# viq854/bwbble

Hardware: AMD Instinct MI355X
Metric: 100bp reads aligned/sec (inexact BWT backward search, IUPAC FM-index) (higher is better)
Workload: dtype u64

## Files before the change

### bwbble_amd/csrc/bwb_hip.hip

```cpp
#include <hip/hip_runtime.h>
#include <time.h>
#include <algorithm>
#include <cctype>
#include <cmath>
#include <cstdio>
#include <cstdlib>
#include <cstring>
#include <memory>
#include <string>
#include <thread>
#include <vector>
#include "../../include/bwbble_hip.h"
#include "bwb_kernels.h"
static double wall_s() { struct timespec ts; clock_gettime(CLOCK_MONOTONIC, &ts); return ts.tv_sec + 1e-9 * ts.tv_nsec; }
#include "bwb_lane.h"

static thread_local std::string g_err;
static int fail(int code, const std::string &m) { g_err = m; return code; }
#define HIPCHK(x)                                                                                         \
	do {                                                                                                  \
		hipError_t e_ = (x);                                                                              \
		if (e_ != hipSuccess) return fail(BWB_E_HIP, std::string(#x) + ": " + hipGetErrorString(e_));  \
	} while (0)

// ... 23 lines not shown
	hipError_t reserve(size_t n) {
		if (p && bytes >= n) return hipSuccess;
		if (p) (void)hipHostFree(p);
		p = nullptr; bytes = 0;
		hipError_t e = hipHostMalloc(&p, n ? n : 1, hipHostMallocDefault);
		if (e == hipSuccess) bytes = n; else p = nullptr;
		return e;
	}
	template <typename T> T *as() const { return (T *)p; }
};
struct Event {
	hipEvent_t e = nullptr;
	Event() = default;
	Event(const Event &) = delete;
	Event &operator=(const Event &) = delete;
	~Event() { if (e) (void)hipEventDestroy(e); }
	hipError_t create() { return e ? hipSuccess : hipEventCreate(&e); }
};

struct AltBufs {
	DevMem d_cnt, d_off, d_bsum, d_alts;
	PinMem h_off, h_alts;
};

struct ScratchClass {
	DevMem mem;
	LaneScratch sc{};
	uint32_t blocks = 0;
	bool ready = false;
};

struct Slot {
	bool uploaded = false, submitted = false, complete = false, fetched = false;
	uint32_t n_reads = 0, stride = 0, maxlen = 0, dstride = 0;
	DevMem d_reads, d_lens, d_dbuf, d_status, d_n, d_off, d_worklist, d_log, d_ctl, d_dbg_iters, d_src;
	uint32_t n_tot = 0;
	bool inherit = false;
	std::vector<uint32_t> h_src;
	uint64_t log_cap = 0;
	PinMem h_reads, h_lens, h_cnt, h_off, h_log, h_ctl;
	DevMem d_place;
	PinMem h_place;
	int placed_mm = -1;
	AltBufs alt;
	int placed_alt = -1;
	std::vector<uint8_t> h_status;
	std::vector<uint64_t> h_aln_off;
	std::vector<bwb_aln> h_alns;
	Event ev_up;
	bool calcd_queued = false;
	Event ev_calcd;
	uint64_t launch = 0;
	uint32_t *ctl_counter() const { return d_ctl.as<uint32_t>(); }
	unsigned int *ctl_done() const { return d_ctl.as<unsigned int>() + 16; }
	unsigned long long *ctl_count() const { return (unsigned long long *)(d_ctl.as<unsigned char>() + 128); }
	uint32_t *ctl_counter2() const { return d_ctl.as<uint32_t>() + 48; }
};

struct PendingTime { hipEvent_t e0, e1; int kind; };

struct bwb_hip_ctx {
	int device = 0, num_cu = 0;
	hipStream_t stream = nullptr, cstream = nullptr, rstream = nullptr;
	hipStream_t dstream = nullptr;
	int calcd_ahead = 0;
	DevIndex ix{};
	DevMem d_buckets, d_SA, d_stats, d_descs, d_misc;
// ... 436 lines not shown
	c->p = *p; c->have_params = true;
	c->kp = KParams{ p->max_diff, p->max_gapo, p->max_gape, p->max_entries, p->mm_score, p->gapo_score, p->gape_score,
	                 p->seed_length, p->max_diff_seed, p->max_best, p->no_indel_length, nb, p->use_precalc ? 1 : 0, p->is_multiref ? 1 : 0 };
	c->wide = wide;

	uint32_t maxlen = 0, n_bad = 0;
	const uint32_t sl = (uint32_t)p->seed_length;
	auto is_source = [&](const uint8_t *seq, uint32_t len) {
		if (!(sl && len > sl) || len > 255) return false;
		if (p->use_precalc) { if (len < PRECALC_LEN) return false; for (int k = 0; k < PRECALC_LEN; k++) if (seq[k] > 3) return false; }
		return true;
	};
	const bool ghost = carry_seq && is_source(carry_seq, carry_len) && n_reads;
	uint32_t last = ghost ? n_reads : NONE32;
	s.inherit = false;
	s.h_src.clear();
	for (uint32_t i = 0; i < n_reads; i++) {
		const bool bad = lens[i] > 255 || lens[i] > stride || (p->use_precalc && lens[i] < PRECALC_LEN);
		if (bad) { n_bad++; continue; }
		maxlen = std::max<uint32_t>(maxlen, lens[i]);
		if (is_source(reads_fwd + (size_t)i * stride, lens[i])) last = i;
		else if (sl && lens[i] <= sl && last != NONE32) {
			if (!s.inherit) { s.h_src.assign(n_reads, NONE32); s.inherit = true; }
			s.h_src[i] = last;
		}
	}
	const bool use_ghost = ghost && s.inherit;
	if (s.inherit && !use_ghost) for (uint32_t i = 0; i < n_reads; i++) if (s.h_src[i] == n_reads) s.h_src[i] = NONE32;
	if (s.inherit) { bool any = false; for (uint32_t v : s.h_src) any |= v != NONE32; s.inherit = any; }
	if (use_ghost) maxlen = std::max<uint32_t>(maxlen, carry_len);
	s.n_tot = n_reads + (use_ghost && s.inherit ? 1u : 0u);
	if (n_bad) fprintf(stderr, "[bwbble_hip] warning: %u read(s) longer than 255 bases%s get an empty alignment record\n", n_bad, p->use_precalc ? " or shorter than 12 (-P)" : "");
	s.n_reads = n_reads; s.stride = std::min<uint32_t>(stride, std::max<uint32_t>(maxlen, 1)); s.maxlen = maxlen;
	s.dstride = REC_BYTES * rec_count(maxlen) + 16;
	const size_t nr = s.n_tot ? s.n_tot : 1;
	HIPCHK(s.d_reads.reserve(nr * s.stride));
	HIPCHK(s.d_lens.reserve(nr * 2));
	HIPCHK(s.d_dbuf.reserve(nr * s.dstride));
	HIPCHK(s.d_status.reserve(nr));
	HIPCHK(s.d_worklist.reserve(nr * 4));
	HIPCHK(s.d_n.reserve(nr * 4));
	HIPCHK(s.d_off.reserve(nr * 8));
	HIPCHK(s.d_ctl.reserve(256));
	HIPCHK(s.h_ctl.reserve(256));
	HIPCHK(s.ev_up.create());
	const uint64_t want = std::max<uint64_t>((uint64_t)nr * 8, 1u << 16);
	if (s.log_cap < want) { HIPCHK(s.d_log.alloc(want * sizeof(bwb_aln))); s.log_cap = want; }
	if (c->dbg_iters) { HIPCHK(s.d_dbg_iters.reserve(nr * 4)); HIPCHK(hipMemsetAsync(s.d_dbg_iters.p, 0, nr * 4, c->cstream)); }
	HIPCHK(s.h_reads.reserve(nr * s.stride));
	HIPCHK(s.h_lens.reserve(nr * 2));
	uint8_t *hr = s.h_reads.as<uint8_t>();
	uint16_t *hl = s.h_lens.as<uint16_t>();
	if (s.stride == stride && !n_bad) { memcpy(hr, reads_fwd, (size_t)n_reads * stride); memcpy(hl, lens, (size_t)n_reads * 2); }
	else
		for (uint32_t i = 0; i < n_reads; i++) {
			const bool bad = lens[i] > 255 || lens[i] > stride || (p->use_precalc && lens[i] < PRECALC_LEN);
			hl[i] = bad ? (uint16_t)BAD_LEN : lens[i];
			memcpy(hr + (size_t)i * s.stride, reads_fwd + (size_t)i * stride, bad ? 0 : lens[i]);
		}
	if (s.n_tot > n_reads) { hl[n_reads] = (uint16_t)carry_len; memcpy(hr + (size_t)n_reads * s.stride, carry_seq, carry_len); }
	if (s.n_tot) {
		HIPCHK(hipMemcpyAsync(s.d_reads.p, hr, (size_t)s.n_tot * s.stride, hipMemcpyHostToDevice, c->cstream));
		HIPCHK(hipMemcpyAsync(s.d_lens.p, hl, (size_t)s.n_tot * 2, hipMemcpyHostToDevice, c->cstream));
	}
	if (s.inherit) {
		HIPCHK(s.d_src.reserve((size_t)n_reads * 4));
		HIPCHK(hipMemcpyAsync(s.d_src.p, s.h_src.data(), (size_t)n_reads * 4, hipMemcpyHostToDevice, c->cstream));
		HIPCHK(hipStreamSynchronize(c->cstream));
	}
	SlotDesc &d = c->h_descs[si];
	d.b.reads = s.d_reads.as<uint8_t>(); d.b.lens = s.d_lens.as<uint16_t>(); d.b.n_reads = n_reads; d.b.stride = s.stride;
	d.b.dbuf = s.d_dbuf.as<uint8_t>(); d.b.dstride = s.dstride; d.b.status = s.d_status.as<uint8_t>(); d.b.dbg_iters = s.d_dbg_iters.as<uint32_t>();
	d.out.alns = s.d_log.as<uint4>(); d.out.count = s.ctl_count(); d.out.cap = s.log_cap; d.out.off = s.d_off.as<uint64_t>(); d.out.n = s.d_n.as<uint32_t>();
	d.done = s.ctl_done();
	HIPCHK(hipMemcpyAsync(c->d_descs.as<SlotDesc>() + si, &d, sizeof(SlotDesc), hipMemcpyHostToDevice, c->cstream));
	HIPCHK(hipEventRecord(s.ev_up.e, c->cstream));
	s.uploaded = true; s.submitted = false; s.complete = false; s.fetched = false; s.placed_mm = -1; s.placed_alt = -1;
	return ensure_class(c, 0);
}

template <typename P> static DTab<P> dtab_of(const bwb_hip_ctx *c) {
	DTab<P> t;
	const bool use = c->dtab_K > 0 && c->dtab_multiref == (c->kp.multiref ? 1 : 0);
	t.ent = use ? c->d_dtab_ent.as<uint4>() : nullptr;
	t.pool = c->d_dtab_pool.as<Intv<P>>();
	t.K = c->dtab_K;
	for (int j = 0; j < 4; j++) t.nm1[j] = c->dtab_nm1[j];
	return t;
}

#define DTAB_MIN_READS 200000u
static bool any_in_flight(const bwb_hip_ctx *c);
template <typename P> static int build_dtab_t(bwb_hip_ctx *c, int K) {
	const double t0 = wall_s();
	ScratchClass &sc = c->cls[0];
	const size_t isz = sizeof(Intv<P>);
	const size_t need_half = std::min<size_t>((size_t)64 << 24, (size_t)(c->ix.length + c->ix.length / 2) + ((size_t)1 << (2 * K))) * isz;
	DevMem tmp;
	unsigned char *pool0 = c->d_pool.as<unsigned char>();
	size_t half = (c->d_pool.bytes / 2) & ~(size_t)255;
	if (half < need_half) {
		if (tmp.alloc(2 * need_half) == hipSuccess) { pool0 = tmp.as<unsigned char>(); half = need_half; }
		else (void)hipGetLastError();
	}
	const unsigned long long cap = half / isz;
// ... 168 lines not shown
		float ms = 0;
		HIPCHK(hipEventElapsedTime(&ms, e0, e1));
		unsigned int hb[POOL_REGIONS * 16], used_max = 0;
		unsigned long long used = 0;
		int rc = fetch(c, hb, bump, sizeof(hb));
		if (rc) return rc;
		const uint32_t priv = (grid + s.sc.n_regions - 1) / s.sc.n_regions * LANE_BLOCK * s.sc.keep;
		for (uint32_t r = 0; r < s.sc.n_regions; r++) { used += std::min(priv + hb[r * 16], s.sc.pool_cap); used_max = std::max(used_max, priv + hb[r * 16]); }
		fprintf(stderr, "[bwb] kl_search class %d slot %d: %u new reads, grid %u, %s%s, %.3f ms, pool chunks used %llu of %d x %u (fullest region asked for %u; %u private per lane)\n",
		        k, si, n_work, grid, suspend ? "slice (parks)" : "drains", resume ? ", resumes parked reads" : "", ms, used, (int)s.sc.n_regions, s.sc.pool_cap, used_max, s.sc.keep);
	}
	if (c->launch_log) return log_launch(c, "kl_search", k, si, !(suspend || slice_iters != 0), c->stream, e0, e1);
	return BWB_OK;
}

static int queue_calc_d(bwb_hip_ctx *c, int si) {
	Slot &s = c->slots[si];
	HIPCHK(s.ev_calcd.create());
	HIPCHK(hipStreamWaitEvent(c->dstream, s.ev_up.e, 0));
	HIPCHK(hipMemsetAsync(s.d_status.p, 0, (size_t)s.n_tot, c->dstream));
	int rc = launch_calc_d(c, 0, si, nullptr, s.n_tot, s.ctl_counter(), nullptr, nullptr, c->dstream);
	if (rc) return rc;
	rc = launch_inherit(c, si, c->dstream);
	if (rc) return rc;
	HIPCHK(hipEventRecord(s.ev_calcd.e, c->dstream));
	s.calcd_queued = true;
	return BWB_OK;
}

static int submit(bwb_hip_ctx *c, int si, bool suspend) {
	Slot &s = c->slots[si];
	if (!s.uploaded) return fail(BWB_E_STATE, "slot_submit: nothing uploaded into this slot");
	if (s.submitted && !s.complete) return fail(BWB_E_STATE, "slot_submit: the slot is still in flight");
	int rc = index_ready(c);
	if (rc) return rc;
	rc = ensure_class(c, 0);
	if (rc) return rc;
	rc = ensure_dtab(c, s.n_reads);
	if (rc) return rc;
	HIPCHK(hipStreamWaitEvent(c->stream, s.ev_up.e, 0));
	const bool ahead = c->calcd_ahead > 0 && s.n_reads != 0;
	if (ahead) {
		if (!s.calcd_queued) { rc = queue_calc_d(c, si); if (rc) return rc; }
		HIPCHK(hipStreamWaitEvent(c->stream, s.ev_calcd.e, 0));
	}
	HIPCHK(hipMemsetAsync(s.d_ctl.p, 0, 256, c->stream));
	s.submitted = true; s.complete = false; s.fetched = false; s.placed_mm = -1; s.placed_alt = -1; s.launch = 0;
	if (s.n_reads == 0) { s.complete = true; s.launch = c->n_launches; return BWB_OK; }
	HIPCHK(hipMemsetAsync(s.d_n.p, 0, (size_t)s.n_reads * 4, c->stream));
	if (!ahead) {
		HIPCHK(hipMemsetAsync(s.d_status.p, 0, (size_t)s.n_tot, c->stream));
		rc = launch_calc_d(c, 0, si, nullptr, s.n_tot, s.ctl_counter(), nullptr, nullptr);
		if (rc) return rc;
		rc = launch_inherit(c, si);
		if (rc) return rc;
	}
	rc = launch_search(c, 0, si, nullptr, s.n_reads, s.ctl_counter(), suspend);
	if (rc) return rc;
	s.launch = c->n_launches;
	for (int k = 1; ahead && k <= c->calcd_ahead; k++) {
		const int sj = (si + k) % BWB_MAX_SLOTS;
		Slot &t = c->slots[sj];
		if (t.uploaded && !t.submitted && !t.calcd_queued && t.n_reads) { rc = queue_calc_d(c, sj); if (rc) return rc; }
	}
	return BWB_OK;
}
// ... 697 lines not shown
```

### bwbble_amd/csrc/bwb_kernels.h

```cpp
#pragma once
#include "bwb_device.h"

#define BWB_BLOCK 256
#define BWB_OCTS_PER_BLOCK 32
#define NONE32 0xFFFFFFFFu
#define BAD_LEN 0xFFFFu
#define ST_OK 0
#define ST_SCRATCH_OVF 1
#define ST_OUT_OVF 2
#define ST_D_OVF 3
#define ST_D_WAIT 4

struct KParams {
	int max_diff, max_gapo, max_gape, max_entries;
	int mm_score, gapo_score, gape_score;
	int seed_length, max_diff_seed, max_best, no_indel_length;
	int num_buckets;
	int use_precalc;
	int multiref;
};

struct Batch {
	const uint8_t *reads;
	const uint16_t *lens;
	uint32_t n_reads, stride;
	uint8_t *dbuf;
	uint32_t dstride;
	uint8_t *status;
	uint32_t *dbg_iters;
};

struct OutBuf {
	uint4 *alns;
	unsigned long long *count;
	uint64_t cap;
	uint64_t *off;
	uint32_t *n;
};

struct SlotDesc {
	Batch b;
	OutBuf out;
	unsigned int *done;
};

struct Work {
	const uint32_t *worklist;
	uint32_t n_work;
	uint32_t *counter;
	uint32_t slot;
	uint32_t suspend;
	uint32_t slice_iters;
	uint32_t resume;
};

enum { STAT_VIS_SINGLE = 0, STAT_VIS_ALPHA, STAT_POPS, STAT_PUSHES, STAT_ALNS, STAT_N, STAT_N_MAX, STAT_VIS_CALCD,
       STAT_BKT_SEARCH , STAT_BKT_CALCD, STAT_PARKED ,
       STAT_ENT_ST , STAT_ENT_LD , STAT_REC_LD ,
       STAT_WAVE_ITERS = 16, STAT_WAVE_ITERS_CALCD = 17, STAT_LOCATE_STEPS = 18 , STAT_STAMPS = 24, STAT_HIST = 40 , STAT_BBPROF = 104 ,
#ifdef BWB_BBPROF
       STAT_WORDS = 104 + 2048 };
#else
       STAT_WORDS = 104 };
#endif

template <typename P> struct Intv { P L, U; };

#define REC_BYTES 16
__host__ __device__ __forceinline__ uint32_t rec_count(uint32_t len) { return (len >> 2) + 1u; }
__device__ __forceinline__ void rec_put(uint8_t *recs, uint32_t nrec, int arr, int k, uint32_t v) {
	const int m = (k + 2) >> 2, t = (k + 2) & 3;
	if ((uint32_t)m < nrec) recs[REC_BYTES * m + arr + t] = (uint8_t)v;
	if (t < 2 && m > 0) recs[REC_BYTES * (m - 1) + arr + 4 + t] = (uint8_t)v;
}
__device__ __forceinline__ uint32_t rec_get(const uint8_t *recs, int arr, int k) { return recs[REC_BYTES * ((k + 2) >> 2) + arr + ((k + 2) & 3)]; }

__device__ __forceinline__ uint32_t single_mask_codes(int c) { return c == 0 ? 1u << 15 : (c == 1 ? 1u << 3 : (c == 2 ? 1u << 7 : 1u << 1)); }
__device__ __forceinline__ uint32_t member_mask(int c) {
	return c == 0 ? 0xFB00u : (c == 1 ? 0x383Cu : (c == 2 ? 0x0BF0u : 0x6266u));
}

template <typename P> __device__ __forceinline__ void load_base(P *s_base, const DevIndex &ix) {
	for (int t = threadIdx.x; t < BWB_BASE_ROWS * 16; t += BWB_BLOCK) s_base[t] = (P)ix.base[t >> 4][t & 15];
	__syncthreads();
}
template <typename P> __device__ __forceinline__ void load_base2(P *s_base, const DevIndex &ix) {
	for (int t = threadIdx.x; t < BWB_BASE_ROWS * 16; t += BWB_BLOCK) {
		const int row = t >> 4, j = t & 15;
		const P v = (P)ix.base[row][j];
		s_base[t] = v;
		if (row < BWB_NSB_MAX) s_base[BWB_BASE_ROWS * 16 + t] = ((0x2A20u >> j) & 1u) ? (P)(ix.base[BWB_ROW_NEG][j] - 1) : v;
	}
	__syncthreads();
}

__global__ void k_relayout(const uint32_t *bwt, const uint64_t *O, uint64_t blk0, uint64_t nblk_chunk, uint64_t nwords_chunk, uint64_t sa0_index,
                           const uint64_t *sbcount , uint4 *buckets) {
	const uint64_t t = (uint64_t)blockIdx.x * blockDim.x + threadIdx.x;
	if (t >= nblk_chunk * 8) return;
	const uint64_t lb = t >> 3, blk = blk0 + lb;
	const int sl = (int)(t & 7);
	const uint64_t w0 = lb * 16;
	uint4 o;
	if (sl < 4) {
		const uint32_t first = w0 < nwords_chunk ? (bwt[w0] >> 28) : 0u;
		const uint64_t *row = O + lb * 16;
		const uint64_t *sb = sbcount + (blk >> BWB_SB_SHIFT) * 16;
		const int cs[4] = { 2 * sl, 2 * sl + 1, 2 * sl + 8, 2 * sl + 9 };
// ... 84 lines not shown
			uint64_t x = (q + u) * 0x9E3779B97F4A7C15ull + seed;
			x ^= x >> 29; x *= 0xBF58476D1CE4E5B9ull; x ^= x >> 32;
			rank_issue<P>(ix.buckets, (P)(ix.length - 1), (P)(x % (ix.length - 1)), ol, rq[u]);
		}
#pragma unroll
		for (int u = 0; u < 4; u++) {
			P v0, v1;
			rank_finish<P, false>(rq[u], s_base, ol, lane, v0, v1);
			acc += (ol == 0 ? 0ull : (unsigned long long)v0) + 3ull * v1;
		}
	}
	acc += __shfl_xor(acc, 1); acc += __shfl_xor(acc, 2); acc += __shfl_xor(acc, 4);
	if (ol == 0 && acc) atomicAdd(checksum, acc);
}

__global__ void k_gather(const uint4 *log, const uint64_t *off, const uint32_t *n, const uint64_t *dst_off, uint32_t n_reads, uint4 *dst) {
	const uint32_t rid = blockIdx.x * (blockDim.x >> 3) + (threadIdx.x >> 3);
	if (rid >= n_reads) return;
	const int ol = threadIdx.x & 7;
	const uint64_t so = off[rid] * 2, d = dst_off[rid] * 2;
	const uint32_t cnt = n[rid] * 2;
	for (uint32_t t = ol; t < cnt; t += 8) dst[d + t] = log[so + t];
}

__global__ void k_dseed_inherit(Batch b, const uint32_t *src, uint32_t n) {
	const uint32_t r = blockIdx.x * blockDim.x + threadIdx.x;
	if (r >= n) return;
	const uint32_t q = src[r];
	if (q == NONE32) return;
	if (b.status[q] == ST_D_OVF) { if (b.status[r] != ST_D_OVF) b.status[r] = ST_D_WAIT; return; }
	const int lr = b.lens[r], lq = b.lens[q];
	uint8_t *rr = b.dbuf + (size_t)r * b.dstride;
	const uint8_t *rq = b.dbuf + (size_t)q * b.dstride;
	for (int k = -2; k < lr; k++) rec_put(rr, rec_count((uint32_t)lr), 8, k, rec_get(rq, 8, k + lq - lr));
	if (b.status[r] == ST_D_WAIT) b.status[r] = ST_OK;
}

__device__ __forceinline__ uint64_t sa_walk(const DevIndex &ix, const uint64_t *s_base, uint64_t sa0_index, uint64_t i, int lane, int ol, uint64_t &j) {
	while ((i & 31) != 0) {
		if (i == sa0_index) { i = 0; j++; continue; }
		RankReq<uint64_t> ra;
		rank_issue<uint64_t>(ix.buckets, ix.length - 1, i, ol, ra);
		const uint4 cq = ra.regular ? ra.q : ix.buckets[(i >> BKT_SHIFT) * 8 + ol];
		const int off = (int)(i & BKT_MASK), srcl = (lane & ~7) + 4 + (off >> 5), bit = off & 31;
		const uint32_t code_here = ((cq.x >> bit) & 1u) | (((cq.y >> bit) & 1u) << 1) | (((cq.z >> bit) & 1u) << 2) | (((cq.w >> bit) & 1u) << 3);
		const uint32_t code = oct_bcast(code_here, srcl);
		uint64_t v0, v1;
		rank_finish<uint64_t, false>(ra, s_base, ol, lane, v0, v1);
		const uint64_t mine = (code & 1u) ? v1 : v0;
		uint64_t nxt = oct_bcast(mine, (lane & ~7) + (int)(code >> 1));
		if (code == 0 && ra.regular && sa0_index >= (i & ~127ull) && sa0_index <= i) nxt--;
		i = nxt;
		j++;
	}
	return i;
}

__global__ __launch_bounds__(BWB_BLOCK) void k_locate(DevIndex ix, const uint64_t *SA, uint64_t sa0_index, const uint64_t *rows, uint64_t n, uint64_t *out, unsigned long long *stats) {
	__shared__ uint64_t s_base[BWB_BASE_ROWS * 16];
	load_base<uint64_t>(s_base, ix);
	const int lane = threadIdx.x & 63, ol = lane & 7;
	const uint64_t noct = (uint64_t)gridDim.x * BWB_OCTS_PER_BLOCK;
	for (uint64_t q = (uint64_t)blockIdx.x * BWB_OCTS_PER_BLOCK + (threadIdx.x >> 3); q < n; q += noct) {
		uint64_t j = 0;
		const uint64_t i = sa_walk(ix, s_base, sa0_index, rows[q], lane, ol, j);
		if (ol == 0) { out[q] = (SA[i >> 5] + j) % ix.length; if (j) atomicAdd(&stats[STAT_LOCATE_STEPS], (unsigned long long)j); }
	}
// ... 223 lines not shown
```

### bwbble_amd/csrc/bwb_lane.h

```cpp
#pragma once
#include "bwb_device.h"
#include "bwb_kernels.h"

#define LANE_BLOCK 256
#ifndef LANE_WAVES_PER_SIMD
#define LANE_WAVES_PER_SIMD 3
#endif
template <typename P> using Lds = __attribute__((address_space(3))) P *;
__device__ __forceinline__ unsigned long long wballot(bool b) { return __builtin_amdgcn_ballot_w64(b); }
__device__ __forceinline__ bool wany(bool b) { return __builtin_amdgcn_ballot_w64(b) != 0ull; }
__device__ __forceinline__ bool wall(bool b) { return __builtin_amdgcn_ballot_w64(!b) == 0ull; }
#define CHUNK_SLOTS 64
#define POOL_REGIONS 8
#define BSTATE_ROW_MIN 128
#define PRECALC_LEN 12
#define ADMIT_CHUNKS 1024
#define SAVE_U4 16
#define ALN_U4 3

struct LaneScratch {
	uint4 *pool;
	size_t region_u4;
	uint32_t n_regions;
	unsigned int *pool_bump;
// ... 419 lines not shown
                                                        uint32_t dbg_ld, uint32_t dbg_lds, unsigned long long *stats, DTab<P> dt) {
	extern __shared__ __align__(16) unsigned char smem_[];
	const LdsBytes smem = (LdsBytes)(uintptr_t)(((uint32_t)(uintptr_t)(LdsBytes)smem_ + 127u) & ~127u);
	P *s_base = (P *)smem;
	const int lane = (int)(threadIdx.x & 63u);
	LdsBytes wlds = smem + CALCD_WAVES_OFF + (threadIdx.x >> 6) * WAVE_LDS_BYTES_NU(CALCD_NU);
	Lds<u32x4> stage = (Lds<u32x4>)wlds, zero_row = (Lds<u32x4>)(smem + CALCD_ZERO_OFF);
	const Lds<P> sb = (Lds<P>)smem;
	if (threadIdx.x < 32) ((Lds<uint32_t>)zero_row)[threadIdx.x] = 0u;
	load_base<P>(s_base, ix);
	const uint32_t slot = blockIdx.x * LANE_BLOCK + threadIdx.x;
	Intv<P> *lbase = (Intv<P> *)sc.lists_d + (size_t)slot * 2 * sc.lcap;
	const int cap = (int)sc.lcap;
	const uint4 *__restrict__ buckets = ix.buckets;
	const P last_row = (P)(ix.length - 1);

	bool active = false, done = false;
	uint32_t rid = 0;
	int len = 0, phase = 0, plen = 0, r = 0, z = 0, s = 0, curT = 0, cursel = 0;
	Intv<P> nxi; nxi.L = nxi.U = 0; bool nxi_valid = false;
	typedef IntvRegs<P> IR;
	typename IR::W g0 = {}, g1 = {}, g2 = {}, g3 = {};
	int cg = -1;
	int c = 4, cnext = 4;
	P cL = 0, cU = 0;
	ListW<P> nx; nx.T = 0; nx.tL = nx.tU = 0; nx.fL = nx.fU = 0;
	ListBuf<P> wb; wb.b0 = wb.b1 = wb.b2 = wb.b3 = typename IntvRegs<P>::W{};
	int32_t nm = 0, prev_nm = 0;
	uint32_t bacc = 0, cntN = 0;
	unsigned long long vis = 0;
	uint32_t r_vis = 0, n_bkt = 0;
	const uint8_t *seq = b.reads;
	const Intv<P> *curb = lbase;
	auto from_table = [&]() -> bool {
		if (!dt.ent || dbgD || r < dt.K) return false;
		unsigned long long idx = 0;
		bool ok = true;
		for (int t = 0; t < dt.K; t++) { const uint32_t ch = seq[r - t]; ok &= ch <= 3u; idx |= (unsigned long long)(ch & 3u) << (2 * t); }
		if (!ok) return false;
		const uint4 ea = dt.ent[2 * idx], eb = dt.ent[2 * idx + 1];
		const int T = (int)dtab_T(ea);
		if (!dtab_valid(ea) || T + 15 > cap) return false;
		uint8_t *rec = b.dbuf + (size_t)rid * b.dstride;
		const uint32_t dbw[3] = { eb.x, eb.y, eb.z };
		for (int t = 0; t < dt.K; t++) {
			const int k = plen - 1 - (r - t);
			const uint32_t tb = (dbw[t >> 2] >> (8 * (t & 3))) & 255u;
			const uint32_t zz = (uint32_t)z + (tb & 127u);
			uint32_t byte = (zz > 127u ? 127u : zz) | (tb & 128u);
			if (t == 0 && k > 0 && dt.nm1[seq[r] & 3u] == (uint32_t)prev_nm) byte |= 128u;
			rec_put(rec, rec_count((uint32_t)len), phase ? 8 : 0, phase ? k + (len - kp.seed_length) : k, byte);
			if (!phase) {
				const int i1 = k + 1;
				bacc |= (uint32_t)seq[len - i1] << (4 * (i1 & 3));
				if ((i1 & 3) == 3 || i1 == len) { *(uint16_t *)(rec + REC_BYTES * (i1 >> 2) + 6) = (uint16_t)bacc; bacc = 0; }
			}
		}
		z += (int)dtab_z(ea); prev_nm = (int32_t)ea.z; nm = 0; r_vis += ea.w;
		curb = dt.pool + dtab_off(ea); curT = T; s = 0; cg = -1; cursel = 0; nx.T = 0;
		{ const Intv<P> tl = curb[T - 1]; cL = tl.L; cU = tl.U; }
		if (T >= 2) nxi = curb[0];
		nxi_valid = T >= 2;
		r -= dt.K; c = seq[r]; cnext = r >= 1 ? seq[r - 1] : 4;
		return true;
	};

	for (;;) {
		if (!active && !done) {
			rid = grab_read(wk);
			if (rid == NONE32) done = true;
			else {
				len = b.lens[rid];
				const bool unrep = len == BAD_LEN;
				if (unrep) len = 0;
				r_vis = 0;
				seq = b.reads + (size_t)rid * b.stride;
				phase = 0; plen = len; r = len - 1; z = 0; s = 0; cursel = 0; nm = 0; prev_nm = 0; bacc = 0; cntN = 0;
				{
					uint4 *rz = (uint4 *)(b.dbuf + (size_t)rid * b.dstride);
					for (uint32_t m = 0; m < rec_count((uint32_t)len); m++) rz[m] = make_uint4(0u, 0u, 0u, m << 16);
				}
				c = len > 0 ? seq[len - 1] : 4; cnext = len > 1 ? seq[len - 2] : 4;
				cL = 0; cU = last_row; curT = 1; nxi_valid = false; cg = -1;
				nx.T = 0; curb = lbase;
				active = len > 0;
				if (!(kp.seed_length && len > kp.seed_length)) {
					uint8_t *rec = b.dbuf + (size_t)rid * b.dstride;
					for (int k = -2; k < len; k++)
						if (k - (len - kp.seed_length) >= 0) rec_put(rec, rec_count((uint32_t)len), 8, k, 0x80u);
				}
				if (active && kp.use_precalc)
					for (int k = 0; k < PRECALC_LEN; k++) if (seq[k] > 3) active = false;
				if (!active) { b.dbuf[(size_t)rid * b.dstride + b.dstride - 4] = 0; b.status[rid] = ST_OK; }
				else (void)from_table();
			}
		}
		if (wall(done)) break;
		P iL = 0, iU = 0;
		const int gq = s & 3;
		const typename IR::W gw = gq == 0 ? g0 : (gq == 1 ? g1 : (gq == 2 ? g2 : g3));
		if (active) {
			if (c > 3 && phase == 0) cntN++;
			if (c <= 3) {
				if (s == curT - 1) { iL = cL; iU = cU; }
				else if (nxi_valid) { iL = nxi.L; iU = nxi.U; }
				else if ((s >> 2) == cg) { iL = IR::lo(gw); iU = IR::hi(gw); }
				else { const Intv<P> v = curb[s]; iL = v.L; iU = v.U; asm volatile("" :: "v"(iL), "v"(iU)); }
			}
		}
		{
			const bool want = active && c <= 3 && s + 1 < curT - 1 && ((s + 1) >> 2) != cg;
			const unsigned long long mw = wballot(want);
			const Intv<P> *g = curb + ((s + 1) & ~3);
			IR::fetch(g0, g, mw); IR::fetch(g1, g + 1, mw); IR::fetch(g2, g + 2, mw); IR::fetch(g3, g + 3, mw);
			cg = want ? (s + 1) >> 2 : cg;
		}
		const bool need = active && c <= 3;
		uint32_t nbk = 0;
		KidCtx<P> kc;
		uint32_t ne = wave_children<P, CALCD_NU>(buckets, last_row, need, iL, iU, false, sb, stage, zero_row, lane, nbk, kc);
		n_bkt += nbk;
		if (!active) { nxi_valid = false; continue; }
		bool ovf = false;
		if (c <= 3) {
			r_vis += (uint32_t)kc.nvis;
			ne &= kp.multiref ? member_mask(c) : single_mask_codes(c);
			if (list_full<P>(nx, cap)) { ovf = true; ne = 0; }
			while (ne) {
				const int j = __ffs((int)ne) - 1;
				ne &= ne - 1;
				P L, U;
				kid_get<P>(kc, sb, j, L, U);
				nm += (int32_t)(uint32_t)(U - L + 1);
				list_add_buf<P>(nx, wb, lbase, cursel ^ 1, L, U, cap);
			}
			s++;
		}
		if (ovf) { b.status[rid] = ST_D_OVF; active = false; nxi_valid = false; continue; }
		if (c > 3 || s >= curT) {
			if (c <= 3) list_flush_buf<P>(nx, wb, lbase, cursel ^ 1, cap);
			cursel ^= 1; curb = lbase + cursel * cap;
			curT = (c > 3) ? 0 : nx.T; cL = nx.tL; cU = nx.tU;
			if (curT >= 2) { nxi.L = nx.fL; nxi.U = nx.fU; }
			nx.T = 0; s = 0; cg = -1;
			const bool restarted = curT == 0;
			if (restarted) {
				cL = 0; cU = last_row; curT = 1; z++;
				nm = (int32_t)(uint32_t)ix.length;
			}
			const int k = plen - 1 - r;
			{
				const uint32_t byte = (uint32_t)((z > 127 ? 127 : z) | ((k > 0 && nm == prev_nm) ? 0x80 : 0));
				uint8_t *rec = b.dbuf + (size_t)rid * b.dstride;
				rec_put(rec, rec_count((uint32_t)len), phase ? 8 : 0, phase ? k + (len - kp.seed_length) : k, byte);
				if (!phase) {
					const int i1 = k + 1;
					bacc |= (uint32_t)c << (4 * (i1 & 3));
					if ((i1 & 3) == 3 || i1 == len) { *(uint16_t *)(rec + REC_BYTES * (i1 >> 2) + 6) = (uint16_t)bacc; bacc = 0; }
				}
			}
			if (dbgD) {
				int32_t *dst = phase ? dbgDs + ((size_t)rid * dbg_lds + k) * 2 : dbgD + ((size_t)rid * dbg_ld + k) * 2;
				dst[0] = z; dst[1] = nm;
			}
			prev_nm = nm; nm = 0; r--;
			if (r >= 0) { c = cnext; cnext = r >= 1 ? seq[r - 1] : 4; }
			if (r < 0) {
				if (dbgD) {
					int32_t *dst = phase ? dbgDs + ((size_t)rid * dbg_lds + plen) * 2 : dbgD + ((size_t)rid * dbg_ld + plen) * 2;
					dst[0] = z + 1; dst[1] = 0;
				}
				if (phase == 0 && kp.seed_length && len > kp.seed_length) {
					phase = 1; plen = kp.seed_length; r = plen - 1; z = 0; prev_nm = 0;
					cL = 0; cU = last_row; curT = 1;
					c = seq[r]; cnext = r >= 1 ? seq[r - 1] : 4;
					(void)from_table();
				} else {
					b.dbuf[(size_t)rid * b.dstride + b.dstride - 4] = (uint8_t)(cntN > 255 ? 255 : cntN);
					*(uint32_t *)(b.dbuf + (size_t)rid * b.dstride + b.dstride - 8) = r_vis;
					b.status[rid] = ST_OK;
					vis += r_vis;
					active = false;
				}
			} else if (restarted) (void)from_table();
		}
		nxi_valid = active && c <= 3 && s == 0 && curT >= 2;
	}
	if (vis) { atomicAdd(&stats[STAT_VIS_SINGLE], vis); atomicAdd(&stats[STAT_VIS_CALCD], vis); }
	if (lane == 0 && n_bkt) atomicAdd(&stats[STAT_BKT_CALCD], (unsigned long long)n_bkt);
}

#ifndef BWB_TEST_POS_BIAS
#define BWB_TEST_POS_BIAS 0ull
#endif
template <typename P> __device__ __forceinline__ P pos_enc(P v) { return sizeof(P) == 8 ? (P)((uint64_t)v + (uint64_t)BWB_TEST_POS_BIAS) : v; }
template <typename P> __device__ __forceinline__ P pos_dec(P v) { return sizeof(P) == 8 ? (P)((uint64_t)v - (uint64_t)BWB_TEST_POS_BIAS) : v; }

template <typename P> struct LEntry {
	P L, U;
	uint32_t f;
	uint32_t sa;
	uint32_t runsLo, runsHi;
	uint32_t runs2Lo, runs2Hi;
};

template <typename P, bool WIDE> struct LHeap {
// ... 225 lines not shown
       H_W1, H_W2, H_W4, H_W8, H_W32, H_W128, H_WBIG, H_NE0, H_NE1, H_NE2, H_NE3_4, H_NE5_8, H_NE9, H_PUSH_GAP, H_PUSH_MIS, H_PUSH_MATCH,
       H_DEL_OK, H_MM_OK, H_INS_OK, H_TOP_RELOAD, H_WAVE_ITERS, H_WAVE_GAPLOOP, H_WAVE_MISLOOP, H_WAVE_MATCHLOOP, H_WAVE_ANY_TWO_BKT, H_WAVE_ANY_WIDE8,
       H_WAVE_NREQ_LE16, H_ALPHA, H_EXACT_MULTI, H_FINISH, H_ALLOC, H_WAVE_ANY_EXACT, H_WAVE_ANY_EXPAND, H_WAVE_ALL_EXACT, H_EXP_SAME_W1, H_EXP_SAME_W2_4, H_PH_GAP, H_PH_MIS, H_PH_POP, H_EXPAND_AFTER_HIT, H_N };

template <typename P, bool WIDE, bool MULTI>
__global__ __launch_bounds__(LANE_BLOCK, LANE_WAVES_PER_SIMD) void kl_search(DevIndex ix, const SlotDesc *__restrict__ descs, Work wk, KParams kp, LaneScratch sc, unsigned long long *stats) {
	struct KArgsT { DevIndex ix; const SlotDesc *descs; Work wk; KParams kp; LaneScratch sc; unsigned long long *stats; };
#define KARGS ({ const __attribute__((address_space(4))) KArgsT *p_ = (const __attribute__((address_space(4))) KArgsT *)__builtin_amdgcn_kernarg_segment_ptr(); asm volatile("" : "+s"(p_)); p_; })
#define R_descs (KARGS->descs)
#define R_wk(f) (KARGS->wk.f)
#define R_stats (KARGS->stats)
#define R_sc(f) (KARGS->sc.f)
	extern __shared__ __align__(16) unsigned char smem_[];
	const LdsBytes smem = (LdsBytes)(uintptr_t)(((uint32_t)(uintptr_t)(LdsBytes)smem_ + 127u) & ~127u);
	P *s_base = (P *)smem;
	const int lane = (int)(threadIdx.x & 63u);
	const uint32_t wave_in_block = (uint32_t)__builtin_amdgcn_readfirstlane((int)(threadIdx.x >> 6));
	LdsBytes wlds = smem + LDS_WAVES_OFF + wave_in_block * WAVE_LDS_BYTES;
	Lds<u32x4> stage = (Lds<u32x4>)wlds, zero_row = (Lds<u32x4>)(smem + LDS_ZERO_OFF);
	const Lds<P> sb = (Lds<P>)smem;
	__shared__ unsigned long long s_blockfree;
	__shared__ unsigned int s_active, s_nfree, s_left;
	__shared__ unsigned int s_need_sum, s_need_cnt;
	if (threadIdx.x == 0) {
		const uint32_t *bs = R_sc(blocksave) + (size_t)blockIdx.x * 4;
		const bool keep = wk.resume != 0;
		s_blockfree = keep ? ~(((unsigned long long)bs[1] << 32) | bs[0]) : ~0ull;
		s_nfree = keep ? bs[2] : 0u;
		s_active = 0; s_left = 0; s_need_sum = 0; s_need_cnt = 0;
	}
	__shared__ unsigned long long s_cnt[LANE_BLOCK / 64];
	if ((threadIdx.x & 63u) == 0) s_cnt[threadIdx.x >> 6] = 0ull;
	__shared__ unsigned long long s_dbuf[BWB_MAX_SLOTS];
	__shared__ unsigned int s_dstride[BWB_MAX_SLOTS];
	if (threadIdx.x < BWB_MAX_SLOTS) { s_dbuf[threadIdx.x] = (unsigned long long)(uintptr_t)descs[threadIdx.x].b.dbuf; s_dstride[threadIdx.x] = descs[threadIdx.x].b.dstride; }
	if (threadIdx.x < 32) ((Lds<uint32_t>)zero_row)[threadIdx.x] = 0u;
	load_base2<P>(s_base, ix);
	const uint32_t slot = blockIdx.x * LANE_BLOCK + threadIdx.x;
	uint32_t slotv = slot;
	typedef __attribute__((address_space(1))) unsigned char *GlobalBytes;
	GlobalBytes sc_lists = (GlobalBytes)sc.lists, sc_alns = (GlobalBytes)sc.alns, sc_bstate = (GlobalBytes)sc.bstate;
	uint32_t sc_lcap = sc.lcap, sc_acap = sc.acap, sc_brow = sc.brow;
	asm volatile("" : "+v"(sc_lists), "+v"(sc_alns), "+v"(sc_bstate), "+v"(sc_lcap), "+v"(sc_acap), "+v"(sc_brow));
	Intv<P> *const lbase = (Intv<P> *)(unsigned char *)sc_lists + (size_t)slotv * 2 * sc_lcap;
#define myalns ((uint4 *)(unsigned char *)sc_alns + (size_t)slotv * sc_acap * ALN_U4)
#define mysave (R_sc(save) + (size_t)slotv * SAVE_U4)
	auto xs = [&]() -> uint32_t * { return (uint32_t *)(mysave + 15); };
	const int lcap = (int)sc_lcap;
	KParams kq = kp;
#ifndef BWB_NO_KQ
	asm volatile("" : "+s"(kq.max_diff), "+s"(kq.max_gapo), "+s"(kq.max_gape), "+s"(kq.max_entries), "+s"(kq.mm_score), "+s"(kq.gapo_score), "+s"(kq.gape_score));
	asm volatile("" : "+s"(kq.seed_length), "+s"(kq.max_diff_seed), "+s"(kq.max_best), "+s"(kq.no_indel_length), "+s"(kq.num_buckets), "+s"(kq.use_precalc));
#endif
	const int nb = kq.num_buckets;
	const uint4 *__restrict__ buckets = ix.buckets;
	const P last_row = (P)(ix.length - 1);

	LHeap<P, WIDE> h;
	const uint32_t region = blockIdx.x % sc.n_regions;
	h.pblk = (uint32_t)__builtin_amdgcn_readfirstlane((int)((blockIdx.x / sc.n_regions) * LANE_BLOCK + (threadIdx.x & ~63u)));
	h.pshared = ((gridDim.x + sc.n_regions - 1) / sc.n_regions) * LANE_BLOCK * sc.keep;
	h.pool = sc.pool + (size_t)region * sc.region_u4; h.pool_bump = sc.pool_bump + region * 16; h.pool_cap = sc.pool_cap; h.bstate = (uint32_t *)(unsigned char *)sc_bstate + (size_t)slotv * sc_brow; h.nslots = sc.nslots;
	h.xhead = NONE32; h.nfree = (Lds<unsigned int>)&s_nfree; h.keep = sc.keep; h.blockfree = (Lds<unsigned long long>)&s_blockfree;
	h.pX = kq.mm_score; h.pGo = kq.gapo_score; h.pGe = kq.gape_score; h.nbk = nb;
	h.pXv = h.pX; h.pGov = h.pGo; h.pGev = h.pGe; h.nbkv = nb;
	if (!WIDE) asm volatile("" : "+v"(h.pXv), "+v"(h.pGov), "+v"(h.pGev), "+v"(h.nbkv));
	h.far = WIDE && (kq.mm_score > 63 || kq.gapo_score > 63 || kq.gape_score > 63);
#ifdef BWB_NO_PHANTOM
// ... 226 lines not shown
			alpha = MULTI && from_pop && (is_group || (rd_max_diff - (int)((e.f >> 8) & 255u) - (int)((e.f >> 16) & 255u) - (int)(e.f >> 24)) != 0);
			iL = e.L; iU = e.U;
		}
		{
			const bool mid = ex & (s != curT - 1), take = mid & nxi_valid;
			iL = take ? nxi.L : iL; iU = take ? nxi.U : iU;
			if (mid & !nxi_valid) {
				const Intv<P> v = (lbase + (cursel ? lcap : 0))[s]; iL = v.L; iU = v.U;
				asm volatile("" :: "v"(iL), "v"(iU));
			}
		}
		if (ex && s + 1 < curT - 1) nxi = (lbase + (cursel ? lcap : 0))[s + 1];
		h.prefetch(pf_top, pf_hdr);

#ifdef BWB_HIST
		HIST(H_POP, active && !exact_mode && (from_pop || finish)); HIST(H_POP_GAPPED, from_pop && ((e.f >> 16) != 0)); HIST(H_POP_FROM_MIRROR, from_pop && h_mirror);
		HIST(H_EXACT_STEP, active && exact_mode); HIST(H_NEED_RANK, need_rank); HIST(H_ALPHA, need_rank && alpha);
		HIST(H_EXACT_MULTI, active && exact_mode && curT > 1); HIST(H_ALLOC, from_pop && is_group);
		const P hw_ = (P)(iU - iL + 1);
		const bool hsame_ = need_rank && ((P)(iL - 1) >> 7) == (iU >> 7) && iL != 0 && iU != last_row;
		HIST(H_SAME_BKT, hsame_); HIST(H_TWO_BKT, need_rank && !hsame_);
		HIST(H_W1, need_rank && hw_ == 1); HIST(H_W2, need_rank && hw_ == 2); HIST(H_W4, need_rank && hw_ > 2 && hw_ <= 4); HIST(H_W8, need_rank && hw_ > 4 && hw_ <= 8);
		HIST(H_W32, need_rank && hw_ > 8 && hw_ <= 32); HIST(H_W128, need_rank && hw_ > 32 && hw_ <= 128); HIST(H_WBIG, need_rank && (hw_ > 128 || hw_ == 0));
		HISTW(H_WAVE_ANY_TWO_BKT, wany(need_rank && !hsame_) ? 1 : 0); HISTW(H_WAVE_ANY_WIDE8, wany(need_rank && (hw_ > 8 || hw_ == 0)) ? 1 : 0);
		HISTW(H_WAVE_ANY_EXACT, wany(active && exact_mode) ? 1 : 0); HISTW(H_WAVE_ANY_EXPAND, wany(from_pop && need_rank) ? 1 : 0);
		HISTW(H_WAVE_ALL_EXACT, wall(!active || exact_mode) ? 1 : 0);
#endif
		STAMP(1);
		uint32_t wd = 0, ws = 0, ne = 0;
		int cr = 4;
		const unsigned long long rmask = wballot(need_rank);
		const int nreq = __popcll(rmask);
		const bool want_rec = need_rank || (from_pop && rd_len < kq.seed_length);
		const bool rec_load = want_rec && (rec.w >> 16) != (uint32_t)(widx >> 2);
		{
			const unsigned long long mr = wballot(rec_load);
			n_rec = (uint32_t)__builtin_amdgcn_readfirstlane((int)(n_rec + (uint32_t)__popcll(mr)));
			{
				const uint32_t sl_ = rd_myslot;
				const unsigned char *rb = (const unsigned char *)(uintptr_t)((Lds<unsigned long long>)&s_dbuf[0])[sl_] + (size_t)rid * ((Lds<unsigned int>)&s_dstride[0])[sl_];
				prefetch128(rec, rb + REC_BYTES * (widx >> 2), mr);
			}
		}
		STAMP(2);
		HISTW(H_WAVE_NREQ_LE16, nreq <= 16 ? 1 : 0);
		KidCtx<P> kc;
		kc.R = (uint32_t)(uintptr_t)stage; kc.baseL = kc.baseU = sb; kc.qL = kc.qU = false; kc.nvis = 0;
		if (nreq > 0) ne = wave_children<P>(buckets, last_row, need_rank, iL, iU, alpha, sb, stage, zero_row, lane, n_bkt, kc);
		__builtin_amdgcn_s_waitcnt(0x0F70);
		h.give_back(pf_free);
		{
			const uint32_t jb = (uint32_t)widx & 3u;
			const uint32_t sel = jb * 0x101u + 0x0c0c0001u;
			wd = __builtin_amdgcn_perm(rec.y, rec.x, sel); ws = __builtin_amdgcn_perm(rec.w, rec.z, sel);
			const int cf = (int)((rec.y >> (16u + 4u * jb)) & 15u);
			cr = cf > 3 ? 4 : 3 - cf;
		}
		STAMP(14);
		const int e_state = (int)(e.sa & 3u);
		const int scX = e_score + h.pXv, scG = e_score + (e_state == STATE_M ? h.pGov : h.pGev);
		const int wG = e_state == STATE_M ? h.side_of(kq.gapo_score) : h.side_of(kq.gape_score);
		if (!MULTI) ne = (((ne >> 15) & 1u) << 1) | (((ne >> 3) & 1u) << 2) | (((ne >> 7) & 1u) << 3) | (((ne >> 1) & 1u) << 4);
		uint32_t st_cnt = 0;
		auto kid = [&](int j, P &L, P &U) { kid_get<P>(kc, sb, MULTI ? j : (int)((0x173Fu >> (4 * (j - 1))) & 15u), L, U); };
		STAMP(3);

		bool exact_step = active && (exact_mode);
		if (from_pop && is_group) {
			uint64_t gr = ((uint64_t)ERUNS_HI << 32) | ERUNS_LO, gr2 = ((uint64_t)ERUNS2_HI << 32) | ERUNS2_LO;
			const int g_run = (int)((e.f >> 16) & 255u) - 1;
			const int g_sh = 16 * (g_run & 3) + 15;
			const bool g_hi = WIDE && g_run >= 4;
#ifdef BWB_NO_GAP_COMBINE
			const bool comb = false;
#else
			const bool comb = (((g_hi ? gr2 : gr) >> g_sh) & 1ull) == 0ull;
#endif
			const int n = __popc(ne) + (comb ? 1 : 0);
			const uint32_t cst_old = h.cst;
			const uint32_t st0 = h.reserve(cst_old, n, ovf, xs);
			if (!ovf && n > 0) {
				if (st0 != cst_old) h.cprev = cst_old;
				const uint32_t sd = (e.sa & 0x3FCu) | (uint32_t)STATE_D;
				uint32_t sx = st0, gm = ne;
				if (comb) {
					u32x4 w0, w1;
					h.pack(e.L, e.U, (e.f & ~255u) | ((e.f - 1u) & 255u), (e.sa & 0x3FCu) | (uint32_t)STATE_I, (uint32_t)gr, (uint32_t)(gr >> 32), w0, w1, (uint32_t)gr2, (uint32_t)(gr2 >> 32));
					h.store_packed(++sx, w0, w1); st_cnt++;
// ... 446 lines not shown
```

Measured before the change: 419,300.

## Pack D-array records into 4-bit nibbles when difference budget is small

Adds a compact record layout in which each 16-byte record holds eight positions of D-values as saturated 3-bit-plus-flag nibbles, instead of four positions of full bytes. It is used whenever max_diff and max_diff_seed are at most 6. Each record load during the search then covers twice as many read positions, which halves record refetches and the per-read D-buffer footprint. The cost is extra unpack arithmetic, a per-slot mode flag read from LDS, and a new state check that rejects a slot if the budgets grow after upload.

```diff
diff --git a/bwbble_amd/csrc/bwb_hip.hip b/bwbble_amd/csrc/bwb_hip.hip
--- a/bwbble_amd/csrc/bwb_hip.hip
+++ b/bwbble_amd/csrc/bwb_hip.hip
@@ -79,7 +79,7 @@
 
 struct Slot {
 	bool uploaded = false, submitted = false, complete = false, fetched = false;
-	uint32_t n_reads = 0, stride = 0, maxlen = 0, dstride = 0;
+	uint32_t n_reads = 0, stride = 0, maxlen = 0, dstride = 0, rec8 = 0;
 	DevMem d_reads, d_lens, d_dbuf, d_status, d_n, d_off, d_worklist, d_log, d_ctl, d_dbg_iters, d_src;
 	uint32_t n_tot = 0;
 	bool inherit = false;
@@ -582,7 +582,8 @@
 	s.n_tot = n_reads + (use_ghost && s.inherit ? 1u : 0u);
 	if (n_bad) fprintf(stderr, "[bwbble_hip] warning: %u read(s) longer than 255 bases%s get an empty alignment record\n", n_bad, p->use_precalc ? " or shorter than 12 (-P)" : "");
 	s.n_reads = n_reads; s.stride = std::min<uint32_t>(stride, std::max<uint32_t>(maxlen, 1)); s.maxlen = maxlen;
-	s.dstride = REC_BYTES * rec_count(maxlen) + 16;
+	s.rec8 = std::max(p->max_diff, p->max_diff_seed) <= REC8_MAX_BUDGET ? 1u : 0u;
+	s.dstride = REC_BYTES * rec_count(maxlen, s.rec8) + 16;
 	const size_t nr = s.n_tot ? s.n_tot : 1;
 	HIPCHK(s.d_reads.reserve(nr * s.stride));
 	HIPCHK(s.d_lens.reserve(nr * 2));
@@ -620,7 +621,7 @@
 	}
 	SlotDesc &d = c->h_descs[si];
 	d.b.reads = s.d_reads.as<uint8_t>(); d.b.lens = s.d_lens.as<uint16_t>(); d.b.n_reads = n_reads; d.b.stride = s.stride;
-	d.b.dbuf = s.d_dbuf.as<uint8_t>(); d.b.dstride = s.dstride; d.b.status = s.d_status.as<uint8_t>(); d.b.dbg_iters = s.d_dbg_iters.as<uint32_t>();
+	d.b.dbuf = s.d_dbuf.as<uint8_t>(); d.b.dstride = s.dstride; d.b.rec8 = s.rec8; d.b.status = s.d_status.as<uint8_t>(); d.b.dbg_iters = s.d_dbg_iters.as<uint32_t>();
 	d.out.alns = s.d_log.as<uint4>(); d.out.count = s.ctl_count(); d.out.cap = s.log_cap; d.out.off = s.d_off.as<uint64_t>(); d.out.n = s.d_n.as<uint32_t>();
 	d.done = s.ctl_done();
 	HIPCHK(hipMemcpyAsync(c->d_descs.as<SlotDesc>() + si, &d, sizeof(SlotDesc), hipMemcpyHostToDevice, c->cstream));
@@ -855,6 +856,7 @@
 	Slot &s = c->slots[si];
 	if (!s.uploaded) return fail(BWB_E_STATE, "slot_submit: nothing uploaded into this slot");
 	if (s.submitted && !s.complete) return fail(BWB_E_STATE, "slot_submit: the slot is still in flight");
+	if (s.rec8 && std::max(c->kp.max_diff, c->kp.max_diff_seed) > REC8_MAX_BUDGET) return fail(BWB_E_STATE, "slot_submit: another slot was uploaded with larger difference budgets since this one: upload it again");
 	int rc = index_ready(c);
 	if (rc) return rc;
 	rc = ensure_class(c, 0);
diff --git a/bwbble_amd/csrc/bwb_kernels.h b/bwbble_amd/csrc/bwb_kernels.h
--- a/bwbble_amd/csrc/bwb_kernels.h
+++ b/bwbble_amd/csrc/bwb_kernels.h
@@ -26,6 +26,7 @@
 	uint32_t n_reads, stride;
 	uint8_t *dbuf;
 	uint32_t dstride;
+	uint32_t rec8;
 	uint8_t *status;
 	uint32_t *dbg_iters;
 };
@@ -66,14 +67,7 @@
 
 template <typename P> struct Intv { P L, U; };
 
-#define REC_BYTES 16
-__host__ __device__ __forceinline__ uint32_t rec_count(uint32_t len) { return (len >> 2) + 1u; }
-__device__ __forceinline__ void rec_put(uint8_t *recs, uint32_t nrec, int arr, int k, uint32_t v) {
-	const int m = (k + 2) >> 2, t = (k + 2) & 3;
-	if ((uint32_t)m < nrec) recs[REC_BYTES * m + arr + t] = (uint8_t)v;
-	if (t < 2 && m > 0) recs[REC_BYTES * (m - 1) + arr + 4 + t] = (uint8_t)v;
-}
-__device__ __forceinline__ uint32_t rec_get(const uint8_t *recs, int arr, int k) { return recs[REC_BYTES * ((k + 2) >> 2) + arr + ((k + 2) & 3)]; }
+#include "bwb_rec.h"
 
 __device__ __forceinline__ uint32_t single_mask_codes(int c) { return c == 0 ? 1u << 15 : (c == 1 ? 1u << 3 : (c == 2 ? 1u << 7 : 1u << 1)); }
 __device__ __forceinline__ uint32_t member_mask(int c) {
@@ -224,7 +218,7 @@
 	const int lr = b.lens[r], lq = b.lens[q];
 	uint8_t *rr = b.dbuf + (size_t)r * b.dstride;
 	const uint8_t *rq = b.dbuf + (size_t)q * b.dstride;
-	for (int k = -2; k < lr; k++) rec_put(rr, rec_count((uint32_t)lr), 8, k, rec_get(rq, 8, k + lq - lr));
+	for (int k = -2; k < lr; k++) rec_put(rr, rec_count((uint32_t)lr, b.rec8), b.rec8, 8, k, rec_get(rq, rec_count((uint32_t)lq, b.rec8), b.rec8, 8, k + lq - lr));
 	if (b.status[r] == ST_D_WAIT) b.status[r] = ST_OK;
 }
 
diff --git a/bwbble_amd/csrc/bwb_lane.h b/bwbble_amd/csrc/bwb_lane.h
--- a/bwbble_amd/csrc/bwb_lane.h
+++ b/bwbble_amd/csrc/bwb_lane.h
@@ -475,6 +475,20 @@
 	uint32_t r_vis = 0, n_bkt = 0;
 	const uint8_t *seq = b.reads;
 	const Intv<P> *curb = lbase;
+	const uint32_t rec8 = b.rec8;
+	uint32_t dacc = 0;
+	auto put_pos = [&](int k, uint32_t byte, uint32_t base) {
+		uint8_t *rec = b.dbuf + (size_t)rid * b.dstride;
+		const uint32_t nrec = rec_count((uint32_t)len, rec8);
+		const int kk = phase ? k + (len - kp.seed_length) : k;
+		if (rec8) {
+			rec8_acc(rec, nrec, phase ? 8 : 0, kk, len - 1, byte, dacc);
+			if (!phase) rec8_acc_base(rec, k + 1, len, base, bacc);
+		} else {
+			rec_put(rec, nrec, 0u, phase ? 8 : 0, kk, byte);
+			if (!phase) rec4_acc_base(rec, k + 1, len, base, bacc);
+		}
+	};
 	auto from_table = [&]() -> bool {
 		if (!dt.ent || dbgD || r < dt.K) return false;
 		unsigned long long idx = 0;
@@ -484,7 +498,6 @@
 		const uint4 ea = dt.ent[2 * idx], eb = dt.ent[2 * idx + 1];
 		const int T = (int)dtab_T(ea);
 		if (!dtab_valid(ea) || T + 15 > cap) return false;
-		uint8_t *rec = b.dbuf + (size_t)rid * b.dstride;
 		const uint32_t dbw[3] = { eb.x, eb.y, eb.z };
 		for (int t = 0; t < dt.K; t++) {
 			const int k = plen - 1 - (r - t);
@@ -492,12 +505,7 @@
 			const uint32_t zz = (uint32_t)z + (tb & 127u);
 			uint32_t byte = (zz > 127u ? 127u : zz) | (tb & 128u);
 			if (t == 0 && k > 0 && dt.nm1[seq[r] & 3u] == (uint32_t)prev_nm) byte |= 128u;
-			rec_put(rec, rec_count((uint32_t)len), phase ? 8 : 0, phase ? k + (len - kp.seed_length) : k, byte);
-			if (!phase) {
-				const int i1 = k + 1;
-				bacc |= (uint32_t)seq[len - i1] << (4 * (i1 & 3));
-				if ((i1 & 3) == 3 || i1 == len) { *(uint16_t *)(rec + REC_BYTES * (i1 >> 2) + 6) = (uint16_t)bacc; bacc = 0; }
-			}
+			put_pos(k, byte, phase ? 0u : (uint32_t)seq[r - t]);
 		}
 		z += (int)dtab_z(ea); prev_nm = (int32_t)ea.z; nm = 0; r_vis += ea.w;
 		curb = dt.pool + dtab_off(ea); curT = T; s = 0; cg = -1; cursel = 0; nx.T = 0;
@@ -518,10 +526,10 @@
 				if (unrep) len = 0;
 				r_vis = 0;
 				seq = b.reads + (size_t)rid * b.stride;
-				phase = 0; plen = len; r = len - 1; z = 0; s = 0; cursel = 0; nm = 0; prev_nm = 0; bacc = 0; cntN = 0;
+				phase = 0; plen = len; r = len - 1; z = 0; s = 0; cursel = 0; nm = 0; prev_nm = 0; bacc = 0; dacc = 0; cntN = 0;
 				{
 					uint4 *rz = (uint4 *)(b.dbuf + (size_t)rid * b.dstride);
-					for (uint32_t m = 0; m < rec_count((uint32_t)len); m++) rz[m] = make_uint4(0u, 0u, 0u, m << 16);
+					for (uint32_t m = 0; m < rec_count((uint32_t)len, rec8); m++) rz[m] = make_uint4(0u, 0u, 0u, rec_init_w(m, rec8));
 				}
 				c = len > 0 ? seq[len - 1] : 4; cnext = len > 1 ? seq[len - 2] : 4;
 				cL = 0; cU = last_row; curT = 1; nxi_valid = false; cg = -1;
@@ -530,7 +538,7 @@
 				if (!(kp.seed_length && len > kp.seed_length)) {
 					uint8_t *rec = b.dbuf + (size_t)rid * b.dstride;
 					for (int k = -2; k < len; k++)
-						if (k - (len - kp.seed_length) >= 0) rec_put(rec, rec_count((uint32_t)len), 8, k, 0x80u);
+						if (k - (len - kp.seed_length) >= 0) rec_put(rec, rec_count((uint32_t)len, rec8), rec8, 8, k, 0x80u);
 				}
 				if (active && kp.use_precalc)
 					for (int k = 0; k < PRECALC_LEN; k++) if (seq[k] > 3) active = false;
@@ -594,13 +602,7 @@
 			const int k = plen - 1 - r;
 			{
 				const uint32_t byte = (uint32_t)((z > 127 ? 127 : z) | ((k > 0 && nm == prev_nm) ? 0x80 : 0));
-				uint8_t *rec = b.dbuf + (size_t)rid * b.dstride;
-				rec_put(rec, rec_count((uint32_t)len), phase ? 8 : 0, phase ? k + (len - kp.seed_length) : k, byte);
-				if (!phase) {
-					const int i1 = k + 1;
-					bacc |= (uint32_t)c << (4 * (i1 & 3));
-					if ((i1 & 3) == 3 || i1 == len) { *(uint16_t *)(rec + REC_BYTES * (i1 >> 2) + 6) = (uint16_t)bacc; bacc = 0; }
-				}
+				put_pos(k, byte, (uint32_t)c);
 			}
 			if (dbgD) {
 				int32_t *dst = phase ? dbgDs + ((size_t)rid * dbg_lds + k) * 2 : dbgD + ((size_t)rid * dbg_ld + k) * 2;
@@ -614,7 +616,7 @@
 					dst[0] = z + 1; dst[1] = 0;
 				}
 				if (phase == 0 && kp.seed_length && len > kp.seed_length) {
-					phase = 1; plen = kp.seed_length; r = plen - 1; z = 0; prev_nm = 0;
+					phase = 1; plen = kp.seed_length; r = plen - 1; z = 0; prev_nm = 0; dacc = 0;
 					cL = 0; cU = last_row; curT = 1;
 					c = seq[r]; cnext = r >= 1 ? seq[r - 1] : 4;
 					(void)from_table();
@@ -906,8 +908,8 @@
 	__shared__ unsigned long long s_cnt[LANE_BLOCK / 64];
 	if ((threadIdx.x & 63u) == 0) s_cnt[threadIdx.x >> 6] = 0ull;
 	__shared__ unsigned long long s_dbuf[BWB_MAX_SLOTS];
-	__shared__ unsigned int s_dstride[BWB_MAX_SLOTS];
-	if (threadIdx.x < BWB_MAX_SLOTS) { s_dbuf[threadIdx.x] = (unsigned long long)(uintptr_t)descs[threadIdx.x].b.dbuf; s_dstride[threadIdx.x] = descs[threadIdx.x].b.dstride; }
+	__shared__ unsigned int s_dstride[BWB_MAX_SLOTS], s_rec8[BWB_MAX_SLOTS];
+	if (threadIdx.x < BWB_MAX_SLOTS) { s_dbuf[threadIdx.x] = (unsigned long long)(uintptr_t)descs[threadIdx.x].b.dbuf; s_dstride[threadIdx.x] = descs[threadIdx.x].b.dstride; s_rec8[threadIdx.x] = descs[threadIdx.x].b.rec8 ? 1u : 0u; }
 	if (threadIdx.x < 32) ((Lds<uint32_t>)zero_row)[threadIdx.x] = 0u;
 	load_base2<P>(s_base, ix);
 	const uint32_t slot = blockIdx.x * LANE_BLOCK + threadIdx.x;
@@ -1200,14 +1202,15 @@
 		const unsigned long long rmask = wballot(need_rank);
 		const int nreq = __popcll(rmask);
 		const bool want_rec = need_rank || (from_pop && rd_len < kq.seed_length);
-		const bool rec_load = want_rec && (rec.w >> 16) != (uint32_t)(widx >> 2);
+		const uint32_t r8_ = ((Lds<unsigned int>)&s_rec8[0])[rd_myslot];
+		const bool rec_load = want_rec && (rec.w >> 16) != rec_tag_of((uint32_t)widx, r8_);
 		{
 			const unsigned long long mr = wballot(rec_load);
 			n_rec = (uint32_t)__builtin_amdgcn_readfirstlane((int)(n_rec + (uint32_t)__popcll(mr)));
 			{
 				const uint32_t sl_ = rd_myslot;
 				const unsigned char *rb = (const unsigned char *)(uintptr_t)((Lds<unsigned long long>)&s_dbuf[0])[sl_] + (size_t)rid * ((Lds<unsigned int>)&s_dstride[0])[sl_];
-				prefetch128(rec, rb + REC_BYTES * (widx >> 2), mr);
+				prefetch128(rec, rb + REC_BYTES * ((uint32_t)widx >> (2u + r8_)), mr);
 			}
 		}
 		STAMP(2);
@@ -1218,10 +1221,9 @@
 		__builtin_amdgcn_s_waitcnt(0x0F70);
 		h.give_back(pf_free);
 		{
-			const uint32_t jb = (uint32_t)widx & 3u;
-			const uint32_t sel = jb * 0x101u + 0x0c0c0001u;
-			wd = __builtin_amdgcn_perm(rec.y, rec.x, sel); ws = __builtin_amdgcn_perm(rec.w, rec.z, sel);
-			const int cf = (int)((rec.y >> (16u + 4u * jb)) & 15u);
+			uint32_t cf_;
+			rec_unpack(rec.x, rec.y, rec.z, rec.w, (uint32_t)widx, wd, ws, cf_);
+			const int cf = (int)cf_;
 			cr = cf > 3 ? 4 : 3 - cf;
 		}
 		STAMP(14);
diff --git a/bwbble_amd/csrc/bwb_rec.h b/bwbble_amd/csrc/bwb_rec.h
--- /dev/null
+++ b/bwbble_amd/csrc/bwb_rec.h
@@ -0,0 +1,85 @@
+#pragma once
+#include <stdint.h>
+
+#if defined(__HIPCC__)
+#define BWB_REC_FN __host__ __device__ __forceinline__
+#else
+#define BWB_REC_FN static inline
+#endif
+
+#define REC_BYTES 16
+#define REC8_MAX_BUDGET 6
+#define REC8_TAG 0x8000u
+#define REC_NO_TAG 0xFFFFu
+
+BWB_REC_FN uint32_t rec_count(uint32_t len, uint32_t rec8) { return (len >> (rec8 ? 3 : 2)) + 1u; }
+BWB_REC_FN uint32_t rec_tag_of(uint32_t i, uint32_t rec8) { return (i >> (2u + rec8)) | (rec8 << 15); }
+BWB_REC_FN uint32_t rec_init_w(uint32_t m, uint32_t rec8) { return (m | (rec8 << 15)) << 16; }
+BWB_REC_FN uint32_t rec8_nib(uint32_t byte) { const uint32_t v = byte & 127u; return (v > 7u ? 7u : v) | ((byte >> 4) & 8u); }
+BWB_REC_FN uint32_t rec8_byte(uint32_t nib) { return (nib & 7u) | ((nib & 8u) << 4); }
+
+BWB_REC_FN void rec_put(uint8_t *recs, uint32_t nrec, uint32_t rec8, int arr, int k, uint32_t v) {
+	if (rec8) {
+		const int m = (k + 2) >> 3, t = (k + 2) & 7;
+		const uint32_t nib = rec8_nib(v);
+		if ((uint32_t)m < nrec) {
+			uint8_t *p = recs + REC_BYTES * m + arr + (t >> 1);
+			*p = (uint8_t)((*p & ~(15u << (4 * (t & 1)))) | (nib << (4 * (t & 1))));
+		}
+		if (t == 0 && m > 0) recs[REC_BYTES * (m - 1) + 12 + (arr >> 3)] = (uint8_t)nib;
+	} else {
+		const int m = (k + 2) >> 2, t = (k + 2) & 3;
+		if ((uint32_t)m < nrec) recs[REC_BYTES * m + arr + t] = (uint8_t)v;
+		if (t < 2 && m > 0) recs[REC_BYTES * (m - 1) + arr + 4 + t] = (uint8_t)v;
+	}
+}
+BWB_REC_FN uint32_t rec_get(const uint8_t *recs, uint32_t nrec, uint32_t rec8, int arr, int k) {
+	if (rec8) {
+		const int m = (k + 2) >> 3, t = (k + 2) & 7;
+		if ((uint32_t)m < nrec) return rec8_byte((recs[REC_BYTES * m + arr + (t >> 1)] >> (4 * (t & 1))) & 15u);
+		return rec8_byte(recs[REC_BYTES * (m - 1) + 12 + (arr >> 3)] & 15u);
+	}
+	const int m = (k + 2) >> 2, t = (k + 2) & 3;
+	return (uint32_t)m < nrec ? recs[REC_BYTES * m + arr + t] : recs[REC_BYTES * (m - 1) + arr + 4 + t];
+}
+
+BWB_REC_FN void rec8_acc(uint8_t *recs, uint32_t nrec, int arr, int k, int k_last, uint32_t v, uint32_t &acc) {
+	const int m = (k + 2) >> 3, t = (k + 2) & 7;
+	const uint32_t nib = rec8_nib(v);
+	acc |= nib << (4 * t);
+	if (t == 0 && m > 0) recs[REC_BYTES * (m - 1) + 12 + (arr >> 3)] = (uint8_t)nib;
+	if ((t == 7 || k == k_last) && (uint32_t)m < nrec) *(uint32_t *)(recs + REC_BYTES * m + arr) = acc;
+	if (t == 7) acc = 0;
+}
+BWB_REC_FN void rec8_acc_base(uint8_t *recs, int i, int len, uint32_t base, uint32_t &bacc) {
+	bacc |= base << (4 * (i & 7));
+	if ((i & 7) == 7 || i == len) { *(uint32_t *)(recs + REC_BYTES * (i >> 3) + 4) = bacc; bacc = 0; }
+}
+BWB_REC_FN void rec4_acc_base(uint8_t *recs, int i, int len, uint32_t base, uint32_t &bacc) {
+	bacc |= base << (4 * (i & 3));
+	if ((i & 3) == 3 || i == len) { *(uint16_t *)(recs + REC_BYTES * (i >> 2) + 6) = (uint16_t)bacc; bacc = 0; }
+}
+
+BWB_REC_FN void rec_unpack(uint32_t x, uint32_t y, uint32_t z, uint32_t w, uint32_t i, uint32_t &wd, uint32_t &ws, uint32_t &cf) {
+	if ((int32_t)w < 0) {
+		const uint32_t sh = 4u * (i & 7u);
+#if defined(__HIP_DEVICE_COMPILE__)
+		const uint32_t pd = __builtin_amdgcn_alignbit(w, x, sh), ps = __builtin_amdgcn_alignbit(w >> 8, z, sh);
+#else
+		const uint32_t pd = (uint32_t)((((uint64_t)w << 32) | x) >> sh), ps = (uint32_t)((((uint64_t)(w >> 8) << 32) | z) >> sh);
+#endif
+		wd = ((pd >> 4) & 7u) | (pd & 0x80u) | ((pd & 7u) << 8) | ((pd & 8u) << 12);
+		ws = ((ps >> 4) & 7u) | (ps & 0x80u) | ((ps & 7u) << 8) | ((ps & 8u) << 12);
+		cf = (y >> sh) & 15u;
+	} else {
+		const uint32_t jb = i & 3u;
+#if defined(__HIP_DEVICE_COMPILE__)
+		const uint32_t sel = jb * 0x101u + 0x0c0c0001u;
+		wd = __builtin_amdgcn_perm(y, x, sel); ws = __builtin_amdgcn_perm(w, z, sel);
+#else
+		const uint32_t pd = (uint32_t)((((uint64_t)y << 32) | x) >> (8u * jb)), ps = (uint32_t)((((uint64_t)w << 32) | z) >> (8u * jb));
+		wd = ((pd >> 8) & 255u) | ((pd & 255u) << 8); ws = ((ps >> 8) & 255u) | ((ps & 255u) << 8);
+#endif
+		cf = (y >> (16u + 4u * jb)) & 15u;
+	}
+}
```

Measured after the change: 427,800, median of 6. About the same (+2.0%).
